# vaultah/replicat

Hardware: AMD Instinct MI355X
Metric: GiB/s chunked, device-resident streams (higher is better)
Workload: dtype u8

## Files before the change

### replicat_amd/build.py

```python
import hashlib
import os
import re
import shutil
import subprocess
import sys

HERE = os.path.dirname(os.path.abspath(__file__))
ROOT = os.path.dirname(HERE)
CSRC = os.path.join(HERE, 'csrc')
LIB = os.path.join(HERE, 'libreplicat_chunker.so')
SOURCES = [os.path.join(CSRC, n) for n in ('kernels.hip', 'capi.cpp', 'blake2b.hip', 'capi_digest.cpp', 'gcm.hip',
                                             'capi_cipher.cpp', 'chacha.hip', 'capi_chacha.cpp', 'cipher_host.cpp')]
HEADERS = [os.path.join(CSRC, n) for n in ('gclmul.h', 'digest_kernels.h', 'capi_internal.h', 'cipher_kernels.h',
                                             'knobs.h', 'diag.h', 'cipher_host.h', 'chacha_kernels.h',
                                             'poly1305_limbs.h')] + [
    os.path.join(ROOT, 'include', n) for n in ('replicat_chunker.h', 'replicat_digest.h', 'replicat_cipher.h')]
ARCH = 'gfx950'
FLAGS = [f'--offload-arch={ARCH}', '-O3', '-std=c++17', '-fPIC', '-shared', '-Wall',
         '-mllvm', '-amdgpu-atomic-optimizer-strategy=None']
_ID_RE = re.compile(rb'RC_BUILD_ID:([0-9a-f]{16})')


def hipcc():
    for cand in (os.environ.get('HIPCC'), '/opt/rocm/bin/hipcc', shutil.which('hipcc')):
        if cand and os.path.exists(cand):
            return cand
    raise RuntimeError('hipcc not found (ROCm 7.x required)')


_COMPILER = {}


def compiler_id():
    if 'id' not in _COMPILER:
        cc = hipcc()
        try:
            banner = subprocess.run([cc, '--version'], capture_output=True, text=True,
                                    timeout=120).stdout
        except (OSError, subprocess.SubprocessError):
            banner = ''
        _COMPILER['id'] = os.path.realpath(cc) + '\n' + banner.strip()
    return _COMPILER['id']


def source_id(extra=()):
    h = hashlib.sha256()
    for p in SOURCES + HEADERS:
        h.update(os.path.relpath(p, ROOT).encode() + b'\0')
        with open(p, 'rb') as f:
            h.update(f.read())
    h.update(' '.join(FLAGS + list(extra)).encode())
    h.update(b'\0' + compiler_id().encode())
    return h.hexdigest()[:16]


def embedded_id(path=LIB):
    try:
        with open(path, 'rb') as f:
            m = _ID_RE.search(f.read())
    except OSError:
        return None
    return m.group(1).decode() if m else None


def stale(path=LIB, extra=()):
    return embedded_id(path) != source_id(extra)


def _compile(out, extra=(), verbose=False):
    bid = source_id(extra)
    cmd = [hipcc(), *FLAGS, *extra, f'-DRC_BUILD_ID="{bid}"', '-I', os.path.join(ROOT, 'include'),
           *SOURCES, '-o', out + '.tmp']
    if verbose:
        print(' '.join(cmd), flush=True)
    subprocess.run(cmd, check=True)
    os.replace(out + '.tmp', out)
    return out


def build(force=False, verbose=False):
    if not force and not stale():
        return LIB
    return _compile(LIB, verbose=verbose)


def build_variant(name, defines, verbose=False):
    out_dir = os.path.join(ROOT, 'diag')
    os.makedirs(out_dir, exist_ok=True)
    out = os.path.join(out_dir, f'lib_{name}.so')
    if stale(out, defines):
        _compile(out, defines, verbose)
    return out


def build_diag(verbose=False):
    out_dir = os.path.join(ROOT, 'diag')
    os.makedirs(out_dir, exist_ok=True)
    srcs = SOURCES + [os.path.join(ROOT, 'scripts', 'gcm_diag.cpp')]
    for name, extra in (('gcm_diag_notrace', []), ('gcm_diag', ['-DRC_GCM_TRACE'])):
        cmd = [hipcc(), f'--offload-arch={ARCH}', '-O3', '-std=c++17', *extra,
               '-I', os.path.join(ROOT, 'include'), *srcs, '-o', os.path.join(out_dir, name)]
        if verbose:
            print(' '.join(cmd), flush=True)
        subprocess.run(cmd, check=True)


if __name__ == '__main__':
    if '--variant' in sys.argv:
        i = sys.argv.index('--variant')
        build_variant(sys.argv[i + 1], [a for a in sys.argv[i + 2:] if a.startswith('-D')], True)
    else:
        build(force='--force' in sys.argv, verbose=True)
    if '--diag' in sys.argv:
        build_diag(verbose=True)
```

### replicat_amd/csrc/diag.h

```cpp
#pragma once

#ifdef RC_PLAIN_LOADS
#define RC_STREAM_LOAD(p) (*(p))
#define RC_DIAG_STREAM_AUX 0
#else
#define RC_STREAM_LOAD(p) __builtin_nontemporal_load(p)
#define RC_DIAG_STREAM_AUX 2
#endif

#ifdef RC_DIAG_NO_SLICE_FENCE
#define RC_DIAG_SLICE_FENCE false
#else
#define RC_DIAG_SLICE_FENCE true
#endif

#ifdef RC_DIAG_GRAB_FAULT
#define RC_DIAG_FORCE_GRAB_STOP() (blockIdx.x == 0 && (threadIdx.x >> 6) == 1)
#else
#define RC_DIAG_FORCE_GRAB_STOP() false
#endif

#ifdef RC_DIAG_TILE_STAMPS
__device__ uint64_t g_tile_stamp[3 * 8192];
#define RC_TILE_STAMP_BEGIN()                                                   \
    const uint64_t diag_stamp0_ = __builtin_amdgcn_s_memrealtime();             \
    uint64_t diag_done_ = 0
#define RC_TILE_STAMP_TILE() (++diag_done_)
#define RC_TILE_STAMP_END(gw)                                                   \
    do {                                                                        \
        if ((gw) < 8192) {                                                      \
            g_tile_stamp[3 * (gw)] = diag_stamp0_;                              \
            g_tile_stamp[3 * (gw) + 1] = __builtin_amdgcn_s_memrealtime();      \
            g_tile_stamp[3 * (gw) + 2] = diag_done_;                            \
        }                                                                       \
    } while (0)
extern "C" int rc_diag_tile_read(uint64_t *out, uint32_t waves) {
    if (waves > 8192) waves = 8192;
    if (hipMemcpyFromSymbol(out, HIP_SYMBOL(g_tile_stamp), 3 * 8 * (size_t)waves) != hipSuccess) return 1;
    static uint64_t zero[3 * 8192];
    return hipMemcpyToSymbol(HIP_SYMBOL(g_tile_stamp), zero, sizeof zero) != hipSuccess;
}
#else
#define RC_TILE_STAMP_BEGIN() \
    do {                      \
    } while (0)
#define RC_TILE_STAMP_TILE() \
    do {                     \
    } while (0)
#define RC_TILE_STAMP_END(gw) \
    do {                      \
    } while (0)
#endif

#ifdef RC_DIAG_STAMPS
#define RC_DIAG_ONLY(...) __VA_ARGS__
__device__ uint64_t g_diag[4096];
__device__ uint32_t g_diag_n;
#define RC_STAMP(tag)                                                                      \
    do {                                                                                   \
        if (st.diag && (threadIdx.x & 63) == 0 && g_diag_n < 4000) {                       \
            g_diag[g_diag_n++] = ((uint64_t)(tag) << 56) | __builtin_amdgcn_s_memrealtime(); \
        }                                                                                  \
    } while (0)
#define RC_LSTAMP(tag)                                                                     \
    do {                                                                                   \
        if (diag && (threadIdx.x & 63) == 0 && g_diag_n < 4000) {                          \
            g_diag[g_diag_n++] = ((uint64_t)(tag) << 56) | __builtin_amdgcn_s_memrealtime(); \
        }                                                                                  \
    } while (0)
extern "C" int rc_diag_read(uint64_t *out, uint32_t cap, uint32_t *n) {
    uint32_t k = 0;
    if (hipMemcpyFromSymbol(&k, HIP_SYMBOL(g_diag_n), 4) != hipSuccess) return 1;
    if (k > cap) k = cap;
    if (k && hipMemcpyFromSymbol(out, HIP_SYMBOL(g_diag), k * 8) != hipSuccess) return 1;
    *n = k;
    const uint32_t z = 0;
    return hipMemcpyToSymbol(HIP_SYMBOL(g_diag_n), &z, 4) != hipSuccess;
}
#else
#define RC_DIAG_ONLY(...)
#define RC_STAMP(tag) \
    do {              \
    } while (0)
#define RC_LSTAMP(tag) \
    do {               \
    } while (0)
#endif
```

### replicat_amd/csrc/kernels.hip

```cpp
#include <hip/hip_runtime.h>
#include <stdint.h>

#include "gclmul.h"
#include "diag.h"

using namespace rc;

namespace {

thread_local char g_launch_err[256];

typedef uint32_t u32x4 __attribute__((ext_vector_type(4)));
typedef __attribute__((address_space(1))) const u32x4 gu32x4;
typedef __attribute__((address_space(1))) const uint32_t gu32;

constexpr int kStreamAux = RC_DIAG_STREAM_AUX;

__device__ __forceinline__ __amdgpu_buffer_rsrc_t tile_rsrc(const uint8_t *base,
                                                             uint32_t bytes = 0xffffffffu) {
    return __builtin_amdgcn_make_buffer_rsrc(const_cast<uint8_t *>(base), 0, bytes, 0x00020000);
}
__device__ __forceinline__ u32x4 ring_load(__amdgpu_buffer_rsrc_t r, uint32_t lane_off, int it) {
    return __builtin_amdgcn_raw_buffer_load_b128(r, lane_off, it * 1024, kStreamAux);
}

__device__ __forceinline__ uint32_t lane_id() { return threadIdx.x & 63; }

__device__ __forceinline__ uint32_t max3_u32(uint32_t a, uint32_t b, uint32_t c) {
    uint32_t r;
    asm("v_max3_u32 %0, %1, %2, %3" : "=v"(r) : "v"(a), "v"(b), "v"(c));
    return r;
}


__device__ __forceinline__ uint64_t lane_u64(uint64_t v, int l) {
    const uint32_t lo = (uint32_t)__builtin_amdgcn_readlane((uint32_t)v, l);
    const uint32_t hi = (uint32_t)__builtin_amdgcn_readlane((uint32_t)(v >> 32), l);
    return ((uint64_t)hi << 32) | lo;
}

typedef __attribute__((address_space(4))) const uint64_t cu64;
__device__ __forceinline__ uint64_t sload(const uint64_t *p) { return *(cu64 *)(p); }
__device__ __forceinline__ const uint8_t *sload_ptr(const uint8_t *const *p) {
    return reinterpret_cast<const uint8_t *>(sload(reinterpret_cast<const uint64_t *>(p)));
}

__device__ __forceinline__ uint32_t ld_u32(const uint8_t *p) {
    return *(gu32 *)(p);
}
__device__ __forceinline__ gu32x4 *as_global_x4(const uint8_t *p) { return (gu32x4 *)(p); }

__device__ __forceinline__ uint64_t full_key(const uint64_t *__restrict__ tl,
                                             const uint64_t *__restrict__ th, uint32_t wlo,
                                             uint32_t whi) {
    return tl[wlo & 255] ^ tl[256 + ((wlo >> 8) & 255)] ^ tl[512 + ((wlo >> 16) & 255)] ^
           tl[768 + (wlo >> 24)] ^ th[whi & 255] ^ th[256 + ((whi >> 8) & 255)] ^
           th[512 + ((whi >> 16) & 255)] ^ th[768 + (whi >> 24)];
}

template <int kCtrl, int kRowMask>
__device__ __forceinline__ uint64_t dpp_u64(uint64_t v) {
    const uint32_t lo = (uint32_t)__builtin_amdgcn_update_dpp((int)(uint32_t)v, (int)(uint32_t)v,
                                                              kCtrl, kRowMask, 0xf, false);
    const uint32_t hi = (uint32_t)__builtin_amdgcn_update_dpp((int)(uint32_t)(v >> 32),
                                                              (int)(uint32_t)(v >> 32), kCtrl,
                                                              kRowMask, 0xf, false);
    return ((uint64_t)hi << 32) | lo;
}

template <int kCtrl, int kRowMask>
__device__ __forceinline__ void best_step(uint64_t &k, uint64_t &j) {
    const uint64_t ko = dpp_u64<kCtrl, kRowMask>(k), jo = dpp_u64<kCtrl, kRowMask>(j);
    if (ko > k || (ko == k && jo < j)) {
        k = ko;
        j = jo;
    }
}

__device__ __forceinline__ void wave_best(uint64_t &k, uint64_t &j) {
    best_step<0x111, 0xf>(k, j);
    best_step<0x112, 0xf>(k, j);
    best_step<0x114, 0xf>(k, j);
    best_step<0x118, 0xf>(k, j);
    best_step<0x142, 0xa>(k, j);
    best_step<0x143, 0xc>(k, j);
    k = lane_u64(k, 63);
    j = lane_u64(j, 63);
}


__shared__ __attribute__((aligned(16))) uint32_t s_tile_lds[kTileLdsBytes / 4];

__device__ __forceinline__ uint32_t pf_lds(uint32_t byte_addr) {
    return *reinterpret_cast<const uint32_t *>(reinterpret_cast<const char *>(s_tile_lds) +
                                               byte_addr);
}

__device__ __forceinline__ void pf_addrs(uint32_t w, uint32_t lb_a, uint32_t lb_b, uint32_t *a) {
    a[0] = __builtin_amdgcn_perm(w, lb_a, 0x0c020400u);
    a[1] = __builtin_amdgcn_perm(w, lb_a, 0x0c020500u) + 128;
    a[2] = __builtin_amdgcn_perm(w, lb_b, 0x0c020600u);
    a[3] = __builtin_amdgcn_perm(w, lb_b, 0x0c020700u) + 128;
}
__device__ __forceinline__ uint32_t pf_gather(const uint32_t *a) {
    return __builtin_amdgcn_bitop3_b32(pf_lds(a[0]), pf_lds(a[1]), pf_lds(a[2]), 0x96) ^ pf_lds(a[3]);
}

__device__ __forceinline__ uint32_t pf_entry(uint32_t w, uint32_t lb_a, uint32_t lb_b) {
    const uint32_t a0 = __builtin_amdgcn_perm(w, lb_a, 0x0c020400u);
    const uint32_t a1 = __builtin_amdgcn_perm(w, lb_a, 0x0c020500u);
    const uint32_t a2 = __builtin_amdgcn_perm(w, lb_b, 0x0c020600u);
    const uint32_t a3 = __builtin_amdgcn_perm(w, lb_b, 0x0c020700u);
    return pf_lds(a0) ^ pf_lds(a1 + 128) ^ pf_lds(a2) ^ pf_lds(a3 + 128);
}

__shared__ __attribute__((aligned(16))) uint32_t s_chain_lds[1024 + 4096];

__device__ __forceinline__ uint32_t pfc_entry(const uint32_t *pf, uint32_t w) {
    return pf[w & 255] ^ pf[256 + ((w >> 8) & 255)] ^ pf[512 + ((w >> 16) & 255)] ^
           pf[768 + (w >> 24)];
}

__device__ __forceinline__ void stage_chain_tables(const KeyTables *tab) {
    const uint32_t nt = blockDim.x;
    const uint32_t *gpf = &tab->pf[0][0];
    for (uint32_t i = threadIdx.x; i < 1024u; i += nt) s_chain_lds[i] = gpf[i];
    uint64_t *full = reinterpret_cast<uint64_t *>(s_chain_lds + 1024);
    const uint64_t *gfull = &tab->tl[0][0];
    for (uint32_t i = threadIdx.x; i < 2048u; i += nt) full[i] = gfull[i];
    __syncthreads();
}

__device__ __forceinline__ void take_best(uint64_t k, uint64_t j, uint64_t &bk, uint64_t &bj) {
    if (k > bk || (k == bk && j < bj)) {
        bk = k;
        bj = j;
    }
}

constexpr int kScanUnroll = 16;
#ifndef RC_CHAIN_SCAN_UNROLL
#define RC_CHAIN_SCAN_UNROLL 4
#endif
constexpr int kChainScanUnroll = RC_CHAIN_SCAN_UNROLL;

template <int kScanUnroll>
__device__ __forceinline__ void scan_ranges(const uint64_t *tl, const uint64_t *th,
                                            const uint8_t *base, uint64_t a0, uint64_t b0,
                                            uint64_t a1, uint64_t b1, uint64_t &bk,
                                            uint64_t &bj) {
    const bool e0 = a0 <= b0, e1 = a1 <= b1;
    if (!e0 && !e1) return;
    if (!e0) a0 = b0 = a1;
    if (!e1) a1 = b1 = a0;
    const uint64_t lane = lane_id();
    for (uint64_t r = 0;; r += 64 * kScanUnroll) {
        const bool live0 = e0 && a0 + r <= b0, live1 = e1 && a1 + r <= b1;
// ... 1560 lines not shown
            for (int k = 0; k < kLaneTasks; ++k) {
                if (k == 0 && first) continue;
                task(jq[k], ra[k], rb[k]);
                lq_load(base, jq[k], ra[k], rb[k], x[k]);
            }
            const uint32_t t16 = (uint32_t)(bk >> 48);
            LaneCand c[kLaneTasks];
#pragma unroll
            for (int k = 0; k < kLaneTasks; ++k) c[k] = lq_scan(pf, x[k], jq[k], ra[k], rb[k], t16);
#pragma unroll
            for (int k = 0; k < kLaneTasks; k += 2)
                lq_fold(tl, th, base, c[k], jq[k], ra[k], rb[k], c[k + 1], jq[k + 1], ra[k + 1],
                        rb[k + 1], bk, bj);
            first = false;
            RC_LSTAMP(3);
        }
        RC_LSTAMP(4);

#pragma unroll 1
        for (int r = 0; r < 2; ++r) {
            const uint32_t sv = r == 0 ? +sc0 : +sc1;
            const uint32_t te = r == 0 ? +te0 : +te1, ra = r == 0 ? +a0 : +a1, rb = r == 0 ? +b0 : +b1;
            uint32_t sa = 1, sb = 0;
            if (sv) {
                const uint32_t qlo = (uint32_t)__builtin_ctz(sv), qhi = 31u - (uint32_t)__builtin_clz(sv);
                sa = max(ra, te * kTileKeys + qlo * kGroupKeys);
                sb = min(rb, te * kTileKeys + (qhi + 1) * kGroupKeys - 1);
            }
            for (uint64_t m = __ballot(sa <= sb); m; m &= m - 1) {
                const int l = __builtin_ctzll(m);
                const uint32_t la = (uint32_t)__builtin_amdgcn_readlane(sa, l);
                const uint32_t lb = (uint32_t)__builtin_amdgcn_readlane(sb, l);
                const uint8_t *lbase = reinterpret_cast<const uint8_t *>(lane_u64((uint64_t)base, l));
                uint64_t ek = 0, ej = ~0ull;
                scan_range<kGroupKeys / 64>(tl, th, lbase, la, lb, ek, ej);
                wave_best(ek, ej);
                if (lane == (uint32_t)l && ek != 0) take_best32(ek, (uint32_t)ej, bk, bj);
                RC_LSTAMP(5);
            }
        }
        RC_LSTAMP(6);

        if (walking) {
            int kind = kStepStop;
            uint64_t c1 = 0, c2 = 0;
            if (argmax) {
                uint32_t idx = bk > 0 ? 4u * (bj - s4) : 0u;
                if (idx < minl) idx = (minl + 3) & ~3u;
                if (idx != 0) {
                    c1 = pos + idx;
                    kind = kStepCut;
                }
            }
            if (kind != kStepCut && !prm.open && !(argmax && rem >= 2ull * maxl)) {
                uint64_t c;
                if (rem <= maxl) c = rem;
                else if (rem < (uint64_t)maxl + minl) c = rem / 2;
                else c = maxl;
                if (c != 0) {
                    c1 = pos + c;
                    kind = kStepTail1;
                    if (c < rem) {
                        c2 = L;
                        kind = kStepTail2;
                    }
                }
            }
            if (kind != kStepStop) {
                if (n < cap) out[n++] = c1;
                else overflow = true;
                if (kind == kStepTail2) {
                    if (n < cap) out[n++] = c2;
                    else overflow = true;
                }
            }
            if (kind != kStepCut || overflow) walking = false;
            pos = c1;
            if (pos >= L || n >= prm.max_steps) walking = false;
        }
    }
    if (mine) counts[s] = overflow ? -1 : (int64_t)n;
}

template <int kCtrl>
__device__ __forceinline__ uint32_t qperm32(uint32_t v) {
    return (uint32_t)__builtin_amdgcn_mov_dpp((int)v, kCtrl, 0xf, 0xf, true);
}
template <int kCtrl>
__device__ __forceinline__ uint64_t qperm64(uint64_t v) {
    return (uint64_t)qperm32<kCtrl>((uint32_t)(v >> 32)) << 32 | qperm32<kCtrl>((uint32_t)v);
}
__device__ __forceinline__ void quad_best32(uint64_t &k, uint32_t &j) {
    {
        const uint64_t ko = qperm64<0xB1>(k);
        const uint32_t jo = qperm32<0xB1>(j);
        if (ko > k || (ko == k && jo < j)) k = ko, j = jo;
    }
    {
        const uint64_t ko = qperm64<0x4E>(k);
        const uint32_t jo = qperm32<0x4E>(j);
        if (ko > k || (ko == k && jo < j)) k = ko, j = jo;
    }
}

struct QuadIter {
    u32x4 v;
    uint32_t p;
};

__device__ __forceinline__ QuadIter qi_load(const uint8_t *base, uint32_t j4, uint32_t a,
                                            uint32_t b) {
    QuadIter x = {u32x4{0u, 0u, 0u, 0u}, 0u};
    if (j4 <= b && j4 + 3 >= a) {
        x.v = *as_global_x4(base + 4ull * j4);
        x.p = ld_u32(base + 4ull * j4 - (j4 ? 4 : 0));
    }
    return x;
}

__device__ __forceinline__ void qi_eval(const uint32_t *pf, const uint64_t *tl, const uint64_t *th,
                                        const uint8_t *base, const QuadIter &x, uint32_t j4,
                                        uint32_t a, uint32_t b, uint32_t t16, uint64_t &lk,
                                        uint32_t &lj) {
    if (!(j4 <= b && j4 + 3 >= a)) return;
    const uint32_t wd[5] = {x.p, x.v.x, x.v.y, x.v.z, x.v.w};
    uint32_t e[5];
#pragma unroll
    for (int k = 0; k < 5; ++k) e[k] = pfc_entry(pf, wd[k]);
    bool have = false, tie = false;
    uint32_t ct = 0, cj = 0, clo = 0, chi = 0;
#pragma unroll
    for (int k = 0; k < 4; ++k) {
        const uint32_t j = j4 + k, t = top16_of(e[k], e[k + 1]);
        const bool in = j >= a && j <= b && t >= t16;
        const bool take = in && (!have || t > ct);
        tie = take ? false : (tie || (in && t == ct));
        ct = take ? t : ct;
        cj = take ? j : cj;
        clo = take ? wd[k] : clo;
        chi = take ? wd[k + 1] : chi;
        have = have || in;
    }
    if (have) take_best32(full_key(tl, th, clo, chi), cj, lk, lj);
    if (tie) {
#pragma unroll 1
        for (uint32_t k = 0; k < 4; ++k) {
            const uint32_t j = j4 + k;
            if (j >= a && j <= b)
                take_best32(full_key(tl, th, ld_u32(base + 4ull * j - 4), ld_u32(base + 4ull * j)), j, lk, lj);
        }
    }
}

constexpr int kQuadTasks = 4;

template <int F>
__global__ __launch_bounds__(256) void rc_quad_chain_kernel(const KeyTables *__restrict__ tab,
                                                            StreamDesc d, uint64_t n_streams,
                                                            ChainParams prm,
                                                            const TileRecord *__restrict__ rec,
                                                            uint64_t *__restrict__ cuts,
                                                            int64_t *__restrict__ counts) {
    static_assert(F % 4 == 0 && kLaneIters == 4, "a quad lane per record row and per iteration");
    if (call_faulted(prm)) {
        fault_counts(counts, n_streams);
        return;
    }
    stage_chain_tables(tab);
    const uint32_t *pf = s_chain_lds;
    const uint64_t *full = reinterpret_cast<const uint64_t *>(s_chain_lds + 1024);
    const uint64_t *tl = full, *th = full + 1024;
    const uint32_t lane = lane_id(), q = lane & 3u;
    const uint64_t gid = ((uint64_t)blockIdx.x * blockDim.x + threadIdx.x) >> 2;
    if (gid - (lane >> 2) >= n_streams) return;
    const bool mine = gid < n_streams;
    const uint64_t s = mine ? gid : n_streams - 1;
    const GroupRecord *grp = prm.grp;
    const uint8_t *base = d.ptr[s];
    const uint64_t L = d.len[s], P = d.last[s];
    const uint64_t tb0 = d.tile_base[s], nt = d.tile_base[s + 1] - tb0;
    uint64_t *out = cuts + d.cut_base[s];
    const uint64_t cap = d.cut_cap[s];
    const uint32_t jmax = L >= 8 ? (uint32_t)((L - 4) / 4) : 0u;
    const uint32_t minl = (uint32_t)prm.min_length, maxl = (uint32_t)prm.max_length;
    const uint32_t T = (uint32_t)prm.window;
    auto gtile = [&](bool use, uint32_t t) -> uint64_t { return use && t < nt ? tb0 + t : prm.n_tiles; };

    uint64_t pos = 0, n = 0;
    bool walking = mine && L > 0 && prm.max_steps > 0, overflow = false;
    RC_DIAG_ONLY(const bool diag = gid < 16 && q == 0;)
    for (;;) {
        if (!__any(walking)) break;
        RC_LSTAMP(1);
        const uint64_t rem = L - pos;
        const bool argmax = (P >= pos && P - pos >= maxl) || rem >= 2ull * maxl;
        const uint32_t s4 = (uint32_t)(pos >> 2);
        const uint32_t ja = s4 + 1, jb = min(s4 + T, jmax);
        const bool win = walking && argmax && T > 0 && ja <= jb;
        const uint32_t t_lo = (ja + kTileKeys - 1) / kTileKeys, t_hi = (jb + 1) / kTileKeys;
        const uint32_t nf = win && t_hi > t_lo ? t_hi - t_lo : 0u;
        const uint32_t a0 = ja, b0 = min(jb, t_lo * kTileKeys - 1), te0 = ja / kTileKeys;
        const uint32_t a1 = t_hi * kTileKeys, b1 = jb, te1 = t_hi;
        bool live0 = win && ja < t_lo * kTileKeys;
        bool live1 = win && t_hi >= t_lo && jb >= a1;

        TileRecord fr[F / 4];
#pragma unroll
        for (int i = 0; i < F / 4; ++i) {
            const uint32_t t = 4 * i + q;
            fr[i] = rec[gtile(t < nf, t_lo + t)];
        }
        const TileRecord r0 = rec[gtile(live0, te0)], r1 = rec[gtile(live1, te1)];
        const GroupRecord g0 = grp[gtile(live0, te0)], g1 = grp[gtile(live1, te1)];
        const bool spec = live0;
        const uint32_t lc = (s4 & 255u) >> 2, qc = (s4 & (kTileKeys - 1)) / kGroupKeys;
        const uint32_t jqc = (s4 & ~(uint32_t)(kGroupKeys - 1)) + 4 * lc;
        QuadIter x[kQuadTasks];
        x[0] = qi_load(base, jqc + 256 * q, spec ? a0 : 1u, spec ? b0 : 0u);

        uint64_t bk = 0;
        uint32_t bj = ~0u;
#pragma unroll
        for (int i = 0; i < F / 4; ++i)
            if (4 * (uint32_t)i + q < nf && fr[i].key != 0) take_best32(fr[i].key, (uint32_t)fr[i].j, bk, bj);
        quad_best32(bk, bj);
        if (live0) {
            const uint32_t rj = (uint32_t)r0.j;
            const bool inr = r0.key != 0 && rj >= a0 && rj <= b0;
            if (inr) take_best32(r0.key, rj, bk, bj);
            if (r0.key == 0 || inr || r0.key < bk) live0 = false;
        }
        if (live1) {
            const uint32_t rj = (uint32_t)r1.j;
            const bool inr = r1.key != 0 && rj >= a1 && rj <= b1;
            if (inr) take_best32(r1.key, rj, bk, bj);
            if (r1.key == 0 || inr || r1.key <= bk) live1 = false;
        }
        uint32_t sc0, sc1;
        RC_LSTAMP(2);
        uint64_t h[kTileGroups], t[kTileGroups];
        lane_groups(live0, g0, te0, a0, b0, (uint32_t)(bk >> 48), prm.hot, h, sc0);
        lane_groups(live1, g1, te1, a1, b1, (uint32_t)(bk >> 48), prm.hot, t, sc1);
        static_assert(kTileGroups == 4, "the task queue below spells out four groups");
        auto any_task = [&]() { return (h[0] | h[1] | h[2] | h[3] | t[0] | t[1] | t[2] | t[3]) != 0; };
        auto task = [&](uint32_t &jq, uint32_t &a, uint32_t &b) {
            int r = -1;
            uint32_t g = 0, l = 0;
#define RC_POP(M, R, Q)                            \
    if (r < 0 && M) {                              \
        l = (uint32_t)__builtin_ctzll(M);          \
        M &= M - 1;                                \
        r = R;                                     \
        g = Q;                                     \
    }
            RC_POP(h[0], 0, 0) RC_POP(h[1], 0, 1) RC_POP(h[2], 0, 2) RC_POP(h[3], 0, 3)
            RC_POP(t[0], 1, 0) RC_POP(t[1], 1, 1) RC_POP(t[2], 1, 2) RC_POP(t[3], 1, 3)
#undef RC_POP
            a = 1, b = 0;
            if (r < 0) return;
            jq = (r ? te1 : te0) * kTileKeys + g * kGroupKeys + 4 * l;
            a = r ? a1 : a0;
            b = r ? b1 : b0;
        };
        bool first = false;
#define RC_FIRST(Q)                                              \
    if (spec && qc == Q && (h[Q] >> lc & 1u)) {                  \
        h[Q] &= ~(1ull << lc);                                   \
        first = true;                                            \
    }
        RC_FIRST(0) RC_FIRST(1) RC_FIRST(2) RC_FIRST(3)
#undef RC_FIRST
        uint32_t jq[kQuadTasks], ra[kQuadTasks], rb[kQuadTasks];
        jq[0] = jqc, ra[0] = first ? a0 : 1u, rb[0] = first ? b0 : 0u;
        for (;;) {
            if (!__any(first || any_task())) break;
            bool used[kQuadTasks];
#pragma unroll
            for (int k = 0; k < kQuadTasks; ++k) {
                if (!(k == 0 && first)) {
                    task(jq[k], ra[k], rb[k]);
                    x[k] = qi_load(base, jq[k] + 256 * q, ra[k], rb[k]);
                }
                used[k] = __any(ra[k] <= rb[k]);
            }
            const uint32_t t16 = (uint32_t)(bk >> 48);
            uint64_t lk = 0;
            uint32_t lj = ~0u;
#pragma unroll
            for (int k = 0; k < kQuadTasks; ++k)
                if (used[k]) qi_eval(pf, tl, th, base, x[k], jq[k] + 256 * q, ra[k], rb[k], t16, lk, lj);
            quad_best32(lk, lj);
            if (lk != 0) take_best32(lk, lj, bk, bj);
            first = false;
            RC_LSTAMP(3);
        }
        RC_LSTAMP(4);

#pragma unroll 1
        for (int r = 0; r < 2; ++r) {
            const uint32_t sv = r == 0 ? +sc0 : +sc1;
            const uint32_t te = r == 0 ? +te0 : +te1, ra_ = r == 0 ? +a0 : +a1, rb_ = r == 0 ? +b0 : +b1;
            uint32_t sa = 1, sb = 0;
            if (sv) {
                const uint32_t qlo = (uint32_t)__builtin_ctz(sv), qhi = 31u - (uint32_t)__builtin_clz(sv);
                sa = max(ra_, te * kTileKeys + qlo * kGroupKeys);
                sb = min(rb_, te * kTileKeys + (qhi + 1) * kGroupKeys - 1);
            }
            for (uint64_t m = __ballot(q == 0 && sa <= sb); m; m &= m - 1) {
                const int l = __builtin_ctzll(m);
                const uint32_t la = (uint32_t)__builtin_amdgcn_readlane(sa, l);
                const uint32_t lb = (uint32_t)__builtin_amdgcn_readlane(sb, l);
                const uint8_t *lbase = reinterpret_cast<const uint8_t *>(lane_u64((uint64_t)base, l));
                uint64_t ek = 0, ej = ~0ull;
                scan_range<kGroupKeys / 64>(tl, th, lbase, la, lb, ek, ej);
                wave_best(ek, ej);
                if ((lane >> 2) == ((uint32_t)l >> 2) && ek != 0) take_best32(ek, (uint32_t)ej, bk, bj);
                RC_LSTAMP(5);
            }
        }
        RC_LSTAMP(6);

        if (walking) {
            int kind = kStepStop;
            uint64_t c1 = 0, c2 = 0;
            if (argmax) {
                uint32_t idx = bk > 0 ? 4u * (bj - s4) : 0u;
                if (idx < minl) idx = (minl + 3) & ~3u;
                if (idx != 0) {
                    c1 = pos + idx;
                    kind = kStepCut;
                }
            }
            if (kind != kStepCut && !prm.open && !(argmax && rem >= 2ull * maxl)) {
                uint64_t c;
                if (rem <= maxl) c = rem;
                else if (rem < (uint64_t)maxl + minl) c = rem / 2;
                else c = maxl;
                if (c != 0) {
                    c1 = pos + c;
                    kind = kStepTail1;
                    if (c < rem) {
                        c2 = L;
                        kind = kStepTail2;
                    }
                }
            }
            if (kind != kStepStop) {
                if (n < cap) {
                    if (q == 0) out[n] = c1;
                    ++n;
                } else {
                    overflow = true;
                }
                if (kind == kStepTail2) {
                    if (n < cap) {
                        if (q == 0) out[n] = c2;
                        ++n;
                    } else {
                        overflow = true;
                    }
                }
            }
            if (kind != kStepCut || overflow) walking = false;
            pos = c1;
            if (pos >= L || n >= prm.max_steps) walking = false;
        }
    }
    if (mine && q == 0) counts[s] = overflow ? -1 : (int64_t)n;
}

constexpr uint64_t kNoMerge = ~0ull;
constexpr int64_t kNeedJoin = -2;

constexpr int kRepairSteps = 64;

template <int R>
__global__ __launch_bounds__(256) void rc_merge_kernel(const KeyTables *__restrict__ tab,
                                                       StreamDesc d, uint64_t n_streams,
                                                       ChainParams prm, uint64_t n_segs,
                                                       const TileRecord *__restrict__ rec,
                                                       uint64_t *__restrict__ scratch,
                                                       const uint64_t *__restrict__ seg_counts,
                                                       uint64_t *__restrict__ seg_merge,
                                                       uint64_t *__restrict__ seg_rcount,
                                                       bool repair) {
    if (call_faulted(prm)) return;
    const uint32_t lane = lane_id();
    const uint64_t q = (uint64_t)blockIdx.x * (blockDim.x >> 6) +
                       __builtin_amdgcn_readfirstlane(threadIdx.x >> 6);
    bool active = q < n_segs;
    uint64_t s = 0, k = 0, na = 0, nb = 0, g = 0, ca = ~0ull;
    uint64_t *A = nullptr;
    uint64_t bv = ~0ull, b_last = 0;
    uint64_t result = kNoMerge;
    if (active) {
        s = find_index(d.seg_base, n_streams + 1, q);
        const uint64_t sb = sload(d.seg_base + s), nseg = sload(d.seg_base + s + 1) - sb;
        k = q - sb;
        active = nseg > 1 && k > 0;
    }
    if (active) {
        A = scratch + sload(d.scratch_base + s) + (k - 1) * prm.seg_cap;
        const uint64_t *B = A + prm.seg_cap;
        ca = seg_counts[q - 1];
        const uint64_t cb = seg_counts[q];
        if (ca != ~0ull && cb != ~0ull) {
            na = ca & ~(1ull << 63);
            nb = cb & ~(1ull << 63);
            g = k * prm.seg_bytes;
            const uint64_t a0 = na > 64 ? na - 64 : 0;
            const uint64_t ai = a0 + lane;
            const uint64_t av = ai < na ? A[ai] : 0;
            bv = lane < nb ? B[lane] : ~0ull;
            b_last = lane_u64(bv, 63);
            uint64_t cm = __ballot(ai < na && av >= g);
            const bool whole = a0 == 0 || !(cm & 1ull);
            for (; whole && cm; cm &= cm - 1) {
                const int l = __builtin_ctzll(cm);
                const uint64_t p = lane_u64(av, l);
                if (p == g) {
                    result = (a0 + l + 1) | (0ull << 32);
                    break;
                }
                const uint64_t hit = __ballot(bv == p);
                if (hit) {
                    result = (a0 + l + 1) | ((uint64_t)(__builtin_ctzll(hit) + 1) << 32);
                    break;
                }
                if (nb > 64 && p > b_last) break;
            }
        }
    }
    const bool need = active && result == kNoMerge && ca != ~0ull && (ca >> 63) == 0 && na > 0 &&
                      nb <= 64 && repair;
    if (__syncthreads_or(need)) {
        stage_chain_tables(tab);
        if (need) {
            const uint32_t *pf = s_chain_lds;
            const uint64_t *full = reinterpret_cast<const uint64_t *>(s_chain_lds + 1024);
            const uint64_t *tl = full, *th = full + 1024;
            const uint32_t lb_a = (lane & 31) * 4, lb_b = lb_a | 0x10000u;
            const ChainStream st = chain_stream(d, s);
            RecCache<R> cache;
            uint64_t n = na, pos = A[na - 1];
            const uint64_t b_end = nb ? lane_u64(bv, (int)nb - 1) : 0;
            bool term = false, over = false, past = false;
            for (int step = 0; step < kRepairSteps && result == kNoMerge && !over; ++step) {
                if (pos >= st.L) {
// ... 610 lines not shown
```

Before: 6890.

## Pool quad tasks across the wave through LDS to balance per-lane work

Replaces the per-quad serial task queue, which evaluated up to four tasks per iteration from the quad's own masks, with a wave-wide pool. Each quad publishes its head and tail group masks, ranges and base pointer to LDS and computes an exclusive prefix over task counts. All 16 quads then pull tasks by global index, evaluate them, and merge the best results back through LDS with wavefront fences. This is meant to remove the imbalance where a few quads with many tasks keep the whole wave looping. It adds LDS traffic, per-task locate arithmetic and fences, and sets launch bounds to four workgroups per CU.

After: 6862. About the same (-0.4%).

```diff
diff --git a/replicat_amd/build.py b/replicat_amd/build.py
--- a/replicat_amd/build.py
+++ b/replicat_amd/build.py
@@ -13,7 +13,7 @@
                                              'capi_cipher.cpp', 'chacha.hip', 'capi_chacha.cpp', 'cipher_host.cpp')]
 HEADERS = [os.path.join(CSRC, n) for n in ('gclmul.h', 'digest_kernels.h', 'capi_internal.h', 'cipher_kernels.h',
                                              'knobs.h', 'diag.h', 'cipher_host.h', 'chacha_kernels.h',
-                                             'poly1305_limbs.h')] + [
+                                             'poly1305_limbs.h', 'quad_pool.h')] + [
     os.path.join(ROOT, 'include', n) for n in ('replicat_chunker.h', 'replicat_digest.h', 'replicat_cipher.h')]
 ARCH = 'gfx950'
 FLAGS = [f'--offload-arch={ARCH}', '-O3', '-std=c++17', '-fPIC', '-shared', '-Wall',
diff --git a/replicat_amd/csrc/diag.h b/replicat_amd/csrc/diag.h
--- a/replicat_amd/csrc/diag.h
+++ b/replicat_amd/csrc/diag.h
@@ -52,6 +52,30 @@
     } while (0)
 #endif
 
+#ifdef RC_DIAG_QUAD_TASKS
+__device__ unsigned long long g_qpool_hist[3][64];
+__device__ __forceinline__ void rc_qpool_count(bool walking, uint32_t q, uint32_t cnt, bool first,
+                                               bool any_first, uint32_t total) {
+    uint32_t m = walking ? cnt + (first ? 1u : 0u) : 0u;
+    for (int o = 32; o; o >>= 1) m = max(m, (uint32_t)__shfl_xor((int)m, o));
+    if (walking && q == 0) atomicAdd(&g_qpool_hist[0][min(cnt, 63u)], 1ull);
+    if ((threadIdx.x & 63) == 0) {
+        atomicAdd(&g_qpool_hist[1][min(m, 63u)], 1ull);
+        atomicAdd(&g_qpool_hist[2][min((any_first ? 1u : 0u) + (total + 15) / 16, 63u)], 1ull);
+    }
+}
+#define RC_QPOOL_COUNT(...) rc_qpool_count(__VA_ARGS__)
+extern "C" int rc_diag_qpool_read(uint64_t *out) {
+    if (hipMemcpyFromSymbol(out, HIP_SYMBOL(g_qpool_hist), 3 * 64 * 8) != hipSuccess) return 1;
+    static unsigned long long zero[3][64];
+    return hipMemcpyToSymbol(HIP_SYMBOL(g_qpool_hist), zero, sizeof zero) != hipSuccess;
+}
+#else
+#define RC_QPOOL_COUNT(...) \
+    do {                    \
+    } while (0)
+#endif
+
 #ifdef RC_DIAG_STAMPS
 #define RC_DIAG_ONLY(...) __VA_ARGS__
 __device__ uint64_t g_diag[4096];
diff --git a/replicat_amd/csrc/kernels.hip b/replicat_amd/csrc/kernels.hip
--- a/replicat_amd/csrc/kernels.hip
+++ b/replicat_amd/csrc/kernels.hip
@@ -3,6 +3,7 @@
 
 #include "gclmul.h"
 #include "diag.h"
+#include "quad_pool.h"
 
 using namespace rc;
 
@@ -1869,10 +1870,39 @@
     }
 }
 
-constexpr int kQuadTasks = 4;
+struct PoolRange {
+    uint32_t a, b, te, t16;
+};
+struct PoolResult {
+    uint64_t k;
+    uint32_t j, pad;
+};
+struct __attribute__((aligned(16))) QuadPoolWave {
+    uint64_t masks[kPoolQuads][kPoolMasks];
+    PoolRange rng[kPoolQuads][2];
+    uint64_t base[kPoolQuads];
+    PoolResult res[kPoolQuads];
+    uint16_t incl[kPoolQuads];
+};
+
+__device__ __forceinline__ void wave_lds_fence() {
+    __builtin_amdgcn_fence(__ATOMIC_RELEASE, "wavefront");
+    __builtin_amdgcn_wave_barrier();
+    __builtin_amdgcn_fence(__ATOMIC_ACQUIRE, "wavefront");
+}
+
+__device__ __forceinline__ uint32_t quad_prefix(uint32_t cnt, uint32_t q) {
+    uint32_t excl = 0;
+#pragma unroll
+    for (int b = 0; b < 6; ++b) {
+        const uint64_t m = __ballot(q == 3 && (cnt >> b & 1u));
+        excl += __builtin_amdgcn_mbcnt_hi((uint32_t)(m >> 32), __builtin_amdgcn_mbcnt_lo((uint32_t)m, 0u)) << b;
+    }
+    return excl;
+}
 
 template <int F>
-__global__ __launch_bounds__(256) void rc_quad_chain_kernel(const KeyTables *__restrict__ tab,
+__global__ __launch_bounds__(256, 4) void rc_quad_chain_kernel(const KeyTables *__restrict__ tab,
                                                             StreamDesc d, uint64_t n_streams,
                                                             ChainParams prm,
                                                             const TileRecord *__restrict__ rec,
@@ -1905,6 +1935,10 @@
 
     uint64_t pos = 0, n = 0;
     bool walking = mine && L > 0 && prm.max_steps > 0, overflow = false;
+    __shared__ QuadPoolWave s_qpool[4];
+    static_assert(sizeof(s_qpool) + sizeof(s_chain_lds) <= 32 * 1024, "five workgroups a CU");
+    QuadPoolWave &pw = s_qpool[threadIdx.x >> 6];
+    if (q == 0) pw.base[lane >> 2] = (uint64_t)base;
     RC_DIAG_ONLY(const bool diag = gid < 16 && q == 0;)
     for (;;) {
         if (!__any(walking)) break;
@@ -1932,8 +1966,7 @@
         const bool spec = live0;
         const uint32_t lc = (s4 & 255u) >> 2, qc = (s4 & (kTileKeys - 1)) / kGroupKeys;
         const uint32_t jqc = (s4 & ~(uint32_t)(kGroupKeys - 1)) + 4 * lc;
-        QuadIter x[kQuadTasks];
-        x[0] = qi_load(base, jqc + 256 * q, spec ? a0 : 1u, spec ? b0 : 0u);
+        const QuadIter x0 = qi_load(base, jqc + 256 * q, spec ? a0 : 1u, spec ? b0 : 0u);
 
         uint64_t bk = 0;
         uint32_t bj = ~0u;
@@ -1958,27 +1991,8 @@
         uint64_t h[kTileGroups], t[kTileGroups];
         lane_groups(live0, g0, te0, a0, b0, (uint32_t)(bk >> 48), prm.hot, h, sc0);
         lane_groups(live1, g1, te1, a1, b1, (uint32_t)(bk >> 48), prm.hot, t, sc1);
-        static_assert(kTileGroups == 4, "the task queue below spells out four groups");
-        auto any_task = [&]() { return (h[0] | h[1] | h[2] | h[3] | t[0] | t[1] | t[2] | t[3]) != 0; };
-        auto task = [&](uint32_t &jq, uint32_t &a, uint32_t &b) {
-            int r = -1;
-            uint32_t g = 0, l = 0;
-#define RC_POP(M, R, Q)                            \
-    if (r < 0 && M) {                              \
-        l = (uint32_t)__builtin_ctzll(M);          \
-        M &= M - 1;                                \
-        r = R;                                     \
-        g = Q;                                     \
-    }
-            RC_POP(h[0], 0, 0) RC_POP(h[1], 0, 1) RC_POP(h[2], 0, 2) RC_POP(h[3], 0, 3)
-            RC_POP(t[0], 1, 0) RC_POP(t[1], 1, 1) RC_POP(t[2], 1, 2) RC_POP(t[3], 1, 3)
-#undef RC_POP
-            a = 1, b = 0;
-            if (r < 0) return;
-            jq = (r ? te1 : te0) * kTileKeys + g * kGroupKeys + 4 * l;
-            a = r ? a1 : a0;
-            b = r ? b1 : b0;
-        };
+        static_assert(kTileGroups == 4 && kPoolMasks == 2 * kTileGroups && kLaneHotMax * kPoolMasks <= kPoolMaxTasks,
+                      "the pool publishes four head and four tail masks of at most kLaneHotMax lanes");
         bool first = false;
 #define RC_FIRST(Q)                                              \
     if (spec && qc == Q && (h[Q] >> lc & 1u)) {                  \
@@ -1987,30 +2001,67 @@
     }
         RC_FIRST(0) RC_FIRST(1) RC_FIRST(2) RC_FIRST(3)
 #undef RC_FIRST
-        uint32_t jq[kQuadTasks], ra[kQuadTasks], rb[kQuadTasks];
-        jq[0] = jqc, ra[0] = first ? a0 : 1u, rb[0] = first ? b0 : 0u;
-        for (;;) {
-            if (!__any(first || any_task())) break;
-            bool used[kQuadTasks];
-#pragma unroll
-            for (int k = 0; k < kQuadTasks; ++k) {
-                if (!(k == 0 && first)) {
-                    task(jq[k], ra[k], rb[k]);
-                    x[k] = qi_load(base, jq[k] + 256 * q, ra[k], rb[k]);
+        const uint32_t t16 = (uint32_t)(bk >> 48);
+        uint32_t cnt = 0;
+#pragma unroll
+        for (int g = 0; g < kTileGroups; ++g) cnt += (uint32_t)__popcll(h[g]) + (uint32_t)__popcll(t[g]);
+        const bool pooled = __any(cnt != 0), any_first = __any(first);
+        uint32_t excl = 0, total = 0;
+        QuadIter xp = {u32x4{0u, 0u, 0u, 0u}, 0u};
+        const uint8_t *pbase = base;
+        uint32_t pj4 = 0, pa = 1, pb = 0, pt16 = 0;
+        auto deal = [&](uint32_t p0) {
+            PoolTask tk;
+            pa = 1, pb = 0;
+            if (pool_locate(pw.incl, pw.masks, p0 + (lane >> 2), tk)) {
+                const PoolRange r = pw.rng[tk.owner][tk.mask >> 2];
+                pbase = reinterpret_cast<const uint8_t *>(pw.base[tk.owner]);
+                pj4 = r.te * kTileKeys + (tk.mask & 3u) * kGroupKeys + 4 * tk.lane + 256 * q;
+                pa = r.a, pb = r.b, pt16 = r.t16;
+            }
+            xp = qi_load(pbase, pj4, pa, pb);
+        };
+        if (pooled) {
+            excl = quad_prefix(cnt, q);
+            total = (uint32_t)__builtin_amdgcn_readlane((int)(excl + cnt), 63);
+            if (q == 0) {
+                const uint32_t o = lane >> 2;
+#pragma unroll
+                for (int g = 0; g < kTileGroups; ++g) pw.masks[o][g] = h[g], pw.masks[o][4 + g] = t[g];
+                pw.rng[o][0] = PoolRange{a0, b0, te0, t16};
+                pw.rng[o][1] = PoolRange{a1, b1, te1, t16};
+                pw.incl[o] = (uint16_t)(excl + cnt);
+            }
+            wave_lds_fence();
+            deal(0);
+        }
+        RC_QPOOL_COUNT(walking, q, cnt, first, any_first, total);
+        uint64_t lk = 0;
+        uint32_t lj = ~0u;
+        if (any_first) qi_eval(pf, tl, th, base, x0, jqc + 256 * q, first ? a0 : 1u, first ? b0 : 0u, t16, lk, lj);
+        RC_LSTAMP(3);
+        if (pooled) {
+            for (uint32_t p0 = 0;;) {
+                uint64_t ek = 0;
+                uint32_t ej = ~0u;
+                qi_eval(pf, tl, th, pbase, xp, pj4, pa, pb, pt16, ek, ej);
+                quad_best32(ek, ej);
+                if (q == 0) pw.res[lane >> 2] = PoolResult{ek, ej, 0u};
+                wave_lds_fence();
+                const uint32_t hi = min(excl + cnt, p0 + kPoolQuads);
+                for (uint32_t i = max(excl, p0) + q; i < hi; i += 4) {
+                    const PoolResult r = pw.res[i - p0];
+                    if (r.k != 0) take_best32(r.k, r.j, lk, lj);
                 }
-                used[k] = __any(ra[k] <= rb[k]);
-            }
-            const uint32_t t16 = (uint32_t)(bk >> 48);
-            uint64_t lk = 0;
-            uint32_t lj = ~0u;
-#pragma unroll
-            for (int k = 0; k < kQuadTasks; ++k)
-                if (used[k]) qi_eval(pf, tl, th, base, x[k], jq[k] + 256 * q, ra[k], rb[k], t16, lk, lj);
-            quad_best32(lk, lj);
-            if (lk != 0) take_best32(lk, lj, bk, bj);
-            first = false;
-            RC_LSTAMP(3);
-        }
+                p0 += kPoolQuads;
+                if (p0 >= total) break;
+                wave_lds_fence();
+                deal(p0);
+                RC_LSTAMP(3);
+            }
+        }
+        quad_best32(lk, lj);
+        if (lk != 0) take_best32(lk, lj, bk, bj);
         RC_LSTAMP(4);
 
 #pragma unroll 1
diff --git a/replicat_amd/csrc/quad_pool.h b/replicat_amd/csrc/quad_pool.h
--- /dev/null
+++ b/replicat_amd/csrc/quad_pool.h
@@ -0,0 +1,58 @@
+#pragma once
+#include <stdint.h>
+
+#if defined(__HIPCC__)
+#define RC_POOL_HD __host__ __device__ __forceinline__
+#else
+#define RC_POOL_HD inline
+#endif
+
+constexpr int kPoolQuads = 16;
+constexpr int kPoolMasks = 8;
+constexpr int kPoolMaxTasks = 32;
+
+struct PoolTask {
+    uint32_t owner;
+    uint32_t mask;
+    uint32_t lane;
+};
+
+RC_POOL_HD uint32_t pool_owner(const uint16_t *incl, uint32_t P) {
+    uint32_t o = 0;
+#if defined(__HIPCC__)
+#pragma unroll
+#endif
+    for (int i = 0; i < kPoolQuads; ++i) o += incl[i] <= P ? 1u : 0u;
+    return o;
+}
+
+RC_POOL_HD bool pool_nth(const uint64_t *masks, uint32_t n, uint32_t &mask, uint32_t &lane) {
+    uint64_t m = 0;
+    uint32_t mi = 0, before = 0;
+    bool found = false;
+#if defined(__HIPCC__)
+#pragma unroll
+#endif
+    for (int i = 0; i < kPoolMasks; ++i) {
+        const uint32_t c = (uint32_t)__builtin_popcountll(masks[i]);
+        const bool here = !found && n < before + c;
+        m = here ? masks[i] : m;
+        mi = here ? (uint32_t)i : mi;
+        n -= here ? before : 0u;
+        found = found || here;
+        before += found ? 0u : c;
+    }
+    if (!found) return false;
+    for (; n; --n) m &= m - 1;
+    mask = mi;
+    lane = (uint32_t)__builtin_ctzll(m);
+    return true;
+}
+
+RC_POOL_HD bool pool_locate(const uint16_t *incl, const uint64_t (*masks)[kPoolMasks], uint32_t P,
+                            PoolTask &t) {
+    const uint32_t o = pool_owner(incl, P);
+    if (o >= (uint32_t)kPoolQuads) return false;
+    t.owner = o;
+    return pool_nth(masks[o], P - (o ? incl[o - 1] : 0u), t.mask, t.lane);
+}
```
